# InternetMaximalism/stark-pure-rust

Measured on AMD Instinct MI355X. Metric: 2^24-pt NTT field-elems/sec, higher is better.
Workload: dtype u32x8 (BN254 Fr)

## Files before the change

### stark-pure-rust_amd/csrc/api.hip

```cpp
#include <new>
#include <string.h>

#include "internal.h"
#include "host_b2s.h"
#include "host_json.h"
#include "blake2s.h"

namespace stark {

stark_status hip_fail(stark_ctx* ctx, hipError_t e, const char* what) {
  if (ctx) {
    ctx->last_error = std::string(what) + ": " + hipGetErrorString(e);
  }
  return e == hipErrorOutOfMemory ? STARK_ERR_OOM : STARK_ERR_HIP;
}

bool poison_on() {
  static const bool on = [] {
    const char* v = getenv("STARK_POISON");
    return v && v[0] == '1';
  }();
  return on;
}
void poison_dev(void* p, size_t bytes) {
// ... 240 lines not shown

uint32_t stark_abi_version(void) { return STARK_ABI_VERSION; }
uint32_t stark_verify_simd_width(void) { return (uint32_t)b2s_paths_width(); }
uint32_t stark_json_simd_width(void) { return (uint32_t)json_simd_width(); }

stark_status stark_ctx_create(int device, stark_ctx** out) {
  if (!out) return STARK_ERR_BAD_ARG;
  *out = nullptr;
  int count = 0;
  if (hipGetDeviceCount(&count) != hipSuccess || device < 0 || device >= count) return STARK_ERR_NO_DEVICE;
  hipDeviceProp_t prop;
  if (hipGetDeviceProperties(&prop, device) != hipSuccess) return STARK_ERR_NO_DEVICE;
  if (strncmp(prop.gcnArchName, "gfx950", 6) != 0) return STARK_ERR_NO_DEVICE;
  stark_ctx* ctx = new (std::nothrow) stark_ctx();
  if (!ctx) return STARK_ERR_OOM;
  ctx->device = device;
  if (hipSetDevice(device) != hipSuccess || hipStreamCreateWithFlags(&ctx->stream, hipStreamNonBlocking) != hipSuccess) {
    delete ctx;
    return STARK_ERR_HIP;
  }
  *out = ctx;
  return STARK_OK;
}

void stark_ctx_destroy(stark_ctx* ctx) {
  if (!ctx) return;
  hipSetDevice(ctx->device);
  hipStreamSynchronize(ctx->stream);
  hipDeviceSynchronize();
  for (auto& kv : ctx->tw) {
    if (kv.second->d_lo) hipFree(kv.second->d_lo);
    if (kv.second->d_full) hipFree(kv.second->d_full);
    if (kv.second->d_full_s) hipFree(kv.second->d_full_s);
    for (hipEvent_t e : kv.second->full_ev)
      if (e) hipEventDestroy(e);
  }
  for (stark_merkle_tree*& t : ctx->trees) {
    stark_merkle_free(t);
    t = nullptr;
  }
  for (stark_merkle_tree* t : ctx->fri_trees) stark_merkle_free(t);
  for (void* p : ctx->pinned)
    if (p) hipHostFree(p);
  for (auto& kv : ctx->ext_idx)
    if (kv.second.ptr) hipFree(kv.second.ptr);
  for (auto& kv : ctx->post_tw) {
    if (kv.second.ptr) hipFree(kv.second.ptr);
    if (kv.second.ev) hipEventDestroy(kv.second.ev);
  }
  if (ctx->staged) hipEventDestroy(ctx->staged);
  if (ctx->ev_aux) hipEventDestroy(ctx->ev_aux);
  if (ctx->aux) hipStreamDestroy(ctx->aux);
  ctx->fri_trees.clear();
  for (DevBuf* b : {&ctx->scratch, &ctx->io, &ctx->io2, &ctx->inv_tmp, &ctx->fri_cols, &ctx->r1cs_arena, &ctx->trace_arena, &ctx->trace_raw, &ctx->fri_misc,
                     &ctx->lde_tmp, &ctx->verify_arena, &ctx->verify_lde, &ctx->ext_idx_tmp, &ctx->spot}) {
    if (b->ptr) hipFree(b->ptr);
    if (b->ev) hipEventDestroy(b->ev);
  }
  hipStreamDestroy(ctx->stream);
  delete ctx;
}

const char* stark_ctx_last_error(const stark_ctx* ctx) { return ctx ? ctx->last_error.c_str() : ""; }

stark_status stark_ctx_set_cache_limit(stark_ctx* ctx, size_t bytes) {
  if (!ctx) return STARK_ERR_BAD_ARG;
// ... 168 lines not shown
```

### stark-pure-rust_amd/csrc/internal.h

```cpp
#pragma once
#include <hip/hip_runtime.h>
#include <stdint.h>
#include <stdio.h>
#include <stdlib.h>

#include <chrono>

#include <functional>
#include <future>
#include <map>
#include <memory>
#include <string>
#include <tuple>
#include <vector>

#include "stark_hip.h"
#include "fp_dev.h"
#include "fp_host.h"
#include "host_pool.h"

namespace stark {

struct PhaseClock {
  bool on;
// ... 10 lines not shown
      return v && v[0] && v[0] != '0';
    }();
    return e;
  }
  void mark(const char* phase) {
    if (!on) return;
    const auto now = std::chrono::steady_clock::now();
    fprintf(stderr, "[stark]   %-28s %8.1f us (at %8.1f)\n", phase,
            std::chrono::duration<double, std::micro>(now - last).count(),
            std::chrono::duration<double, std::micro>(now - t0).count());
    last = now;
  }
};

struct DevBuf {
  void* ptr = nullptr;
  size_t bytes = 0;
  hipEvent_t ev = nullptr;
  hipStream_t last = nullptr;
};

struct Twiddles {
  uint32_t log_n = 0, kb = 0;
  fe* d_lo = nullptr;
  fe* d_hi = nullptr;
  fe* d_small = nullptr;
  fe* d_t16 = nullptr;
  fe* d_hi_s = nullptr;
  fe* d_t16_s = nullptr;
  uint32_t l16 = 0;
  uint32_t small_off[16] = {0};
  fe* d_full = nullptr;
  fe* d_full_s = nullptr;
  uint64_t full_used = 0, full_s_used = 0;
  hipEvent_t full_ev[2] = {nullptr, nullptr};
  hipStream_t full_fill[2] = {nullptr, nullptr};
  size_t base_bytes = 0;
  size_t n_small_pairs = 0;
  uint32_t* d_db = nullptr;
  uint32_t db_off[16] = {0};
  HostFp root;
  HostFp inv_n;
};

struct CacheBuf {
  void* ptr = nullptr;
  size_t bytes = 0;
  uint64_t used = 0;
  bool in_use = false;
  hipEvent_t ev = nullptr;
  hipStream_t fill = nullptr;
};

constexpr size_t kDefaultCacheLimit = (size_t)4 << 30;

}

struct stark_ctx {
  int device = 0;
  hipStream_t stream = nullptr;
  std::string last_error;
  stark::DevBuf scratch;
  stark::DevBuf io;
  stark::DevBuf io2;
  stark::DevBuf fri_cols;
  stark::DevBuf r1cs_arena;
  stark::DevBuf trace_arena;
  stark::DevBuf trace_raw;
  stark::DevBuf lde_tmp;
  stark::DevBuf verify_arena, verify_lde;
  stark::DevBuf ext_idx_tmp;
  stark::DevBuf inv_tmp;
  stark::DevBuf spot;
// ... 342 lines not shown
```

### stark-pure-rust_amd/csrc/ntt.hip

```cpp
#include <stdlib.h>

#include "fe_db.h"
#include "internal.h"

namespace stark {

struct ColTw {
  const fe* t16;
  const fe* lo;
  const fe* hi;
  const fe* full;
  uint32_t l16, kb;
  const fe* post;
};


__device__ __forceinline__ void shoup2(fe& r, fe& s, const fe& a, const fe& w, const fe& wq, const fe& c,
                                       const fe& x, const fe& xq) {
  r = fe_mul_shoup(a, w, wq);
  s = fe_mul_shoup(c, x, xq);
}
__device__ __forceinline__ void mul2(fe& r, fe& s, const fe& a, const fe& b, const fe& c, const fe& d) {
  fe_mul_lazy2(r, s, a, b, c, d);
}

__device__ __forceinline__ void bfly_lt2p(fe& x, fe& y, const fe& t) {
  fe_bfly_lazy_reduced(x, y, t);
}

__device__ __forceinline__ void sub2p(fe& t) {
  const P2Limbs q = p2_vgprs();
  asm("v_sub_co_u32 %0, vcc, %0, %8\n\t"
      "v_subb_co_u32 %1, vcc, %1, %9, vcc\n\t"
      "v_subb_co_u32 %2, vcc, %2, %10, vcc\n\t"
      "v_subb_co_u32 %3, vcc, %3, %11, vcc\n\t"
      "v_subb_co_u32 %4, vcc, %4, %12, vcc\n\t"
      "v_subb_co_u32 %5, vcc, %5, %13, vcc\n\t"
      "v_subb_co_u32 %6, vcc, %6, %14, vcc\n\t"
      "v_subb_co_u32 %7, vcc, %7, %15, vcc"
      : "+v"(t.w[0]), "+v"(t.w[1]), "+v"(t.w[2]), "+v"(t.w[3]), "+v"(t.w[4]), "+v"(t.w[5]), "+v"(t.w[6]),
        "+v"(t.w[7])
      : "v"(q.l[0]), "v"(q.l[1]), "v"(q.l[2]), "v"(q.l[3]), "v"(q.l[4]), "v"(q.l[5]), "v"(q.l[6]), "v"(q.l[7])
      : "vcc");
}
__device__ __forceinline__ void csub2p_top(fe& t) {
  if (t.w[7] > STARK_2P7) sub2p(t);
}
template <bool FAST>
__device__ __forceinline__ void bfly(fe& x, fe& y, const fe& t) {
  if (FAST) {
    csub2p_top(x);
    fe_bfly_lazy_reduced(x, y, t);
  } else {
    fe_bfly_lazy(x, y, t);
  }
}
template <bool FAST>
__device__ __forceinline__ void csub2p_t(fe& t) {
  if (FAST) csub2p_top(t);
  fe_csub2p(t);
}
template <bool FAST>
__device__ __forceinline__ void reduce_full(fe& t) {
  csub2p_t<FAST>(t);
  fe_reduce_once(t);
}

__device__ __forceinline__ const uint32_t* dbt(const uint32_t* sdb, uint32_t k) {
  return static_cast<const uint32_t*>(__builtin_assume_aligned(sdb + 72 * k + 4 * (k >> 3), 16));
}

enum : int { kColNone = 0, kColFull = 1, kColT16 = 2, kColTwoLevel = 3, kColSparse = 4 };

constexpr uint32_t kTileLog = 10;
constexpr uint32_t kPassThreads = (1u << kTileLog) / 4;

template <int LOG_R, int COL>
struct DbPlan {
  static constexpr bool on = LOG_R >= 4 && LOG_R <= 8;
  static constexpr bool four = LOG_R == 8 || (LOG_R == 7 && COL == kColSparse);
  static constexpr int s_end = on ? LOG_R - 2 : 0;
  static constexpr uint32_t stride = 4;
  static constexpr uint32_t entries = (on && !four) ? (1u << LOG_R) / (2 * stride) : 0;
  static constexpr uint32_t lds_fe = entries * 9 + entries / 16;
  static constexpr bool last = on && !four && LOG_R <= 7;
  static constexpr uint32_t full_entries = last ? (1u << LOG_R) / 2 : 0;
  static constexpr uint32_t full_fe = full_entries * 9 + full_entries / 16;
  static constexpr uint32_t shoup_fe = last ? 0 : four ? 2 * (1u << LOG_R) : (1u << LOG_R);
  static constexpr int occupancy = on ? 3 : 4;
};

typedef unsigned int u32x4_nt __attribute__((ext_vector_type(4)));
__device__ __forceinline__ fe fe_load_nt(const fe* p) {
  const u32x4_nt* q = reinterpret_cast<const u32x4_nt*>(p);
  const u32x4_nt lo = __builtin_nontemporal_load(q), hi = __builtin_nontemporal_load(q + 1);
  fe r;
  r.w[0] = lo.x; r.w[1] = lo.y; r.w[2] = lo.z; r.w[3] = lo.w;
  r.w[4] = hi.x; r.w[5] = hi.y; r.w[6] = hi.z; r.w[7] = hi.w;
  return r;
}
__device__ __forceinline__ void fe_store_nt(fe* p, const fe& v) {
  u32x4_nt* q = reinterpret_cast<u32x4_nt*>(p);
  __builtin_nontemporal_store(u32x4_nt{v.w[0], v.w[1], v.w[2], v.w[3]}, q);
  __builtin_nontemporal_store(u32x4_nt{v.w[4], v.w[5], v.w[6], v.w[7]}, q + 1);
}

struct XImage {
  fe* base;
  uint32_t n;
  __device__ __forceinline__ fe ld(uint32_t i) const {
    const uint4* v = reinterpret_cast<const uint4*>(base);
    const uint4 lo = v[i], hi = v[n + i];
    fe r;
    r.w[0] = lo.x; r.w[1] = lo.y; r.w[2] = lo.z; r.w[3] = lo.w;
    r.w[4] = hi.x; r.w[5] = hi.y; r.w[6] = hi.z; r.w[7] = hi.w;
    return r;
  }
  __device__ __forceinline__ void st(uint32_t i, const fe& x) const {
    uint4* v = reinterpret_cast<uint4*>(base);
    v[i] = make_uint4(x.w[0], x.w[1], x.w[2], x.w[3]);
    v[n + i] = make_uint4(x.w[4], x.w[5], x.w[6], x.w[7]);
  }
};

template <int LOG_R, int COL>
__global__ __launch_bounds__(kPassThreads, (DbPlan<LOG_R, COL>::occupancy)) void ntt_pass_kernel(
    const fe* __restrict__ in, fe* __restrict__ out, uint32_t log_n, uint32_t log_ns, uint32_t log_b, ColTw ct,
    const fe* __restrict__ small, const uint32_t* __restrict__ db, fe scale, int do_scale, uint32_t log_tiles,
    uint32_t total_tiles, Sparse sp) {
  constexpr uint32_t R = 1u << LOG_R;
  using DB = DbPlan<LOG_R, COL>;
  constexpr bool FAST = LOG_R == 6;
  extern __shared__ __attribute__((aligned(16))) fe lds[];
  fe* sm = lds;
  uint32_t* sdb = reinterpret_cast<uint32_t*>(lds + DB::shoup_fe);
  fe* X = lds + DB::shoup_fe + DB::lds_fe;
  const uint32_t B = 1u << log_b;
  const XImage XI{X, B << LOG_R};
  const uint32_t nthr = (B << LOG_R) >> 2;
  const uint32_t tid = threadIdx.x;
  const bool active = tid < nthr;
  const uint32_t log_cols = log_n - LOG_R;
  const size_t ns_mask = ((size_t)1 << log_ns) - 1;
  const uint32_t tile_mask = (1u << log_tiles) - 1;
  const uint32_t tile = blockIdx.x;
  if (tile >= total_tiles) return;

  uint32_t eb[4], er[4];
#pragma unroll
  for (int t = 0; t < 4; ++t) {
    const uint32_t e = tid + (uint32_t)t * nthr;
    eb[t] = e & (B - 1);
    er[t] = e >> log_b;
  }
  const uint32_t b = tid & (B - 1);
  const uint32_t q = tid >> log_b;

  const uint32_t live_rows = R >> sp.skip, nz_rows = R >> sp.zero_log;
  const uint32_t log_in = sp.zero_log ? sp.log_in : log_n;
  fe v[4];
  if (active) {
    const fe* src = in + ((size_t)(tile >> log_tiles) << log_in) + ((size_t)(tile & tile_mask) << log_b);
#pragma unroll
    for (int t = 0; t < 4; ++t)
      v[t] = er[t] < nz_rows ? fe_load(src + eb[t] + ((size_t)er[t] << log_cols)) : fe_zero();
  }

  {
    constexpr uint32_t kSm = 2 * DB::shoup_fe, kDb = DB::on ? DB::entries * 18 : 0;
    const uint4* db4 = reinterpret_cast<const uint4*>(db);
    const uint4* small4 = reinterpret_cast<const uint4*>(small);
    uint4* sm4 = reinterpret_cast<uint4*>(sm);
    uint4* sdb4 = reinterpret_cast<uint4*>(sdb);
    auto db_src = [&](uint32_t k) { const uint32_t e = k / 18; return (e * DB::stride) * 18 + (k - e * 18); };
    auto db_dst = [&](uint32_t k) { return k + ((k / 18) >> 3); };
    if (blockDim.x == kPassThreads) {
      constexpr uint32_t nSm = (kSm + kPassThreads - 1) / kPassThreads, nDb = (kDb + kPassThreads - 1) / kPassThreads;
      auto in_sm = [&](uint32_t i) { return (i + 1) * kPassThreads <= kSm || tid + i * kPassThreads < kSm; };
      auto in_db = [&](uint32_t i) { return (i + 1) * kPassThreads <= kDb || tid + i * kPassThreads < kDb; };
      uint4 ts[nSm ? nSm : 1], td[nDb ? nDb : 1];
#pragma unroll
      for (uint32_t i = 0; i < nSm; ++i)
        if (in_sm(i)) ts[i] = small4[tid + i * kPassThreads];
#pragma unroll
      for (uint32_t i = 0; i < nDb; ++i)
        if (in_db(i)) td[i] = db4[db_src(tid + i * kPassThreads)];
#pragma unroll
      for (uint32_t i = 0; i < nSm; ++i)
        if (in_sm(i)) sm4[tid + i * kPassThreads] = ts[i];
#pragma unroll
      for (uint32_t i = 0; i < nDb; ++i)
        if (in_db(i)) sdb4[db_dst(tid + i * kPassThreads)] = td[i];
    } else {
      for (uint32_t k = tid; k < kSm; k += blockDim.x) sm4[k] = small4[k];
      for (uint32_t k = tid; k < kDb; k += blockDim.x) sdb4[db_dst(k)] = db4[db_src(k)];
    }
  }
  const size_t boff = (size_t)(tile >> log_tiles) << log_n;
  const size_t j0 = (size_t)(tile & tile_mask) << log_b;

  if (active) {
    if (COL != kColNone && COL != kColSparse) {
      const uint32_t lnr = log_ns + LOG_R;
      fe tw[4];
      if (COL == kColFull) {
#pragma unroll
        for (int t = 0; t < 4; ++t) tw[t] = fe_load_nt(ct.full + ((((j0 + eb[t]) & ns_mask) << LOG_R) + er[t]));
        mul2(v[0], v[1], v[0], tw[0], v[1], tw[1]);
        mul2(v[2], v[3], v[2], tw[2], v[3], tw[3]);
      } else if (COL == kColT16) {
        const fe* e[4];
#pragma unroll
        for (int t = 0; t < 4; ++t) {
          const uint64_t k = ((uint64_t)((j0 + eb[t]) & ns_mask) * er[t]) & (((uint64_t)1 << lnr) - 1);
          e[t] = ct.t16 + 2 * (k << (ct.l16 - lnr));
        }
        shoup2(v[0], v[1], v[0], e[0][0], e[0][1], v[1], e[1][0], e[1][1]);
        shoup2(v[2], v[3], v[2], e[2][0], e[2][1], v[3], e[3][0], e[3][1]);
      } else {
        const uint32_t unit = log_n - lnr;
#pragma unroll
        for (int t = 0; t < 4; ++t) {
          const uint64_t ex = ((uint64_t)((j0 + eb[t]) & ns_mask) * er[t]) << unit;
          tw[t] = fe_mul(ct.lo[ex & (((uint64_t)1 << ct.kb) - 1)], ct.hi[ex >> ct.kb]);
        }
        mul2(v[0], v[1], v[0], tw[0], v[1], tw[1]);
        mul2(v[2], v[3], v[2], tw[2], v[3], tw[3]);
// ... 1 lines not shown
    }
    if (sp.skip == 0) {
      if ((LOG_R & 1) == 0) {
        bfly_lt2p(v[0], v[2], v[2]);
        bfly_lt2p(v[1], v[3], v[3]);
        fe t3;
        if (DB::on) {
          t3 = fe_mul_db(v[3], db + 72u * (1u << (LOG_R - 2)));
        } else {
          const uint32_t ic = 2 * (1u << (LOG_R - 2));
          t3 = fe_mul_shoup(v[3], small[ic], small[ic + 1]);
        }
        fe_csub2p(v[1]);
        bfly<FAST>(v[0], v[1], v[1]);
        bfly<FAST>(v[2], v[3], t3);
      } else {
        bfly_lt2p(v[0], v[2], v[2]);
        bfly_lt2p(v[1], v[3], v[3]);
      }
#pragma unroll
      for (int t = 0; t < 4; ++t) {
        const uint32_t rr = __builtin_bitreverse32(er[t]) >> (32 - LOG_R);
        XI.st((rr << log_b) + eb[t], v[t]);
      }
    } else {
#pragma unroll
      for (int t = 0; t < 4; ++t) {
        if (er[t] >= live_rows) continue;
        const uint32_t rr = __builtin_bitreverse32(er[t]) >> (32 - LOG_R);
        for (uint32_t k = 0; k < (1u << sp.skip); ++k) XI.st(((rr + k) << log_b) + eb[t], v[t]);
      }
    }
  }
  __syncthreads();

  int s = sp.skip ? (int)sp.skip : (LOG_R & 1) ? 1 : 2;
  constexpr int kS0 = (LOG_R & 1) ? 1 : 2;
  if (LOG_R >= 5 && s == kS0) {
    if (active) {
      const uint32_t lq = LOG_R + log_b - 2 - kS0;
      const uint32_t jj = tid >> lq;
      const uint32_t rest = tid & ((1u << lq) - 1);
      const uint32_t i0 = ((((rest >> log_b) << (kS0 + 2)) + jj) << log_b) + (rest & (B - 1));
      const uint32_t st = (1u << kS0) << log_b;
      fe x0 = XI.ld(i0), x1 = XI.ld(i0 + st), x2 = XI.ld(i0 + 2 * st), x3 = XI.ld(i0 + 3 * st);
      if (jj == 0) {
        csub2p_t<FAST>(x1);
        csub2p_t<FAST>(x3);
        bfly<FAST>(x0, x1, x1);
        bfly<FAST>(x2, x3, x3);
        fe t3;
        if (DB::on) {
          t3 = fe_mul_db(x3, db + 72u * (1u << (LOG_R - 2)));
        } else {
          const uint32_t ic = 2 * (1u << (LOG_R - 2));
          t3 = fe_mul_shoup(x3, sm[ic], sm[ic + 1]);
        }
        csub2p_t<FAST>(x2);
        bfly<FAST>(x0, x2, x2);
        bfly<FAST>(x1, x3, t3);
      } else if (DB::on && DB::s_end > kS0 && lq >= 6) {
        const uint32_t ju = __builtin_amdgcn_readfirstlane(jj);
        const uint32_t* wa = db + 72u * (ju << (LOG_R - 1 - kS0));
        const fe t1 = fe_mul_db(x1, wa);
        fe t3 = fe_mul_db(x3, wa);
        bfly<FAST>(x0, x1, t1);
// ... 5 lines not shown
      } else if (DB::on && DB::s_end > kS0) {
        constexpr uint32_t S = DB::stride;
        auto tab = [&](uint32_t e) { return DB::four ? db + 72u * e : dbt(sdb, e / S); };
        const uint32_t* wa = tab(jj << (LOG_R - 1 - kS0));
        const fe t1 = fe_mul_db(x1, wa);
        fe t3 = fe_mul_db(x3, wa);
        bfly<FAST>(x0, x1, t1);
        bfly<FAST>(x2, x3, t3);
        const fe t2 = fe_mul_db(x2, tab(jj << (LOG_R - 2 - kS0)));
        t3 = fe_mul_db(x3, tab((jj + (1u << kS0)) << (LOG_R - 2 - kS0)));
        bfly<FAST>(x0, x2, t2);
        bfly<FAST>(x1, x3, t3);
      } else {
        fe t1, t3;
        const uint32_t ia = 2 * (jj << (LOG_R - 1 - kS0));
        const fe ta = sm[ia], taq = sm[ia + 1];
        shoup2(t1, t3, x1, ta, taq, x3, ta, taq);
        bfly<FAST>(x0, x1, t1);
        bfly<FAST>(x2, x3, t3);
        const uint32_t ic = 2 * ((jj + (1u << kS0)) << (LOG_R - 2 - kS0));
        const fe tc = sm[ic], tcq = sm[ic + 1];
        const uint32_t ib = 2 * (jj << (LOG_R - 2 - kS0));
        const fe t2 = fe_mul_shoup(x2, sm[ib], sm[ib + 1]);
        t3 = fe_mul_shoup(x3, tc, tcq);
        bfly<FAST>(x0, x2, t2);
        bfly<FAST>(x1, x3, t3);
      }
      XI.st(i0, x0);
      XI.st(i0 + 2 * st, x2);
      XI.st(i0 + st, x1);
      XI.st(i0 + 3 * st, x3);
    }
    __syncthreads();
    s = kS0 + 2;
  }
  bool kept = false;
  fe yl[4];
  constexpr uint32_t LT = LOG_R >= 4 ? LOG_R - 4 : 0;
  if (DB::four && s == (int)LT) {
    if (active) {
      const uint32_t t = q & ((1u << LT) - 1), a = q >> LT;
      const uint32_t i0 = (((a << (LT + 2)) + t) << log_b) + b, st = (1u << LT) << log_b;
      fe x[4];
      const bool unit0 = ((64u >> log_b) <= (1u << LT) ? __builtin_amdgcn_readfirstlane(a) : a) == 0;
#pragma unroll
      for (int k = 0; k < 4; ++k) {
        const fe v = XI.ld(i0 + k * st);
        if (k == 0 && unit0) {
          x[0] = v;
          fe_csub2p(x[0]);
          continue;
        }
        const uint32_t e = (__builtin_bitreverse32((a << 2) + k) >> 28) * t;
        x[k] = fe_mul_shoup(v, sm[2 * e], sm[2 * e + 1]);
      }
      bfly_lt2p(x[0], x[1], x[1]);
      bfly_lt2p(x[2], x[3], x[3]);
      const fe t3 = fe_mul_db(x[3], db + 72u * (1u << (LOG_R - 2)));
      fe_csub2p(x[2]);
      bfly<FAST>(x[0], x[2], x[2]);
      bfly<FAST>(x[1], x[3], t3);
#pragma unroll
      for (int k = 0; k < 4; ++k) XI.st(i0 + k * st, x[k]);
    }
    __syncthreads();
    if (active) {
      const uint32_t i0 = (q << log_b) + b, st = (R / 4) << log_b;
      fe x0 = XI.ld(i0), x1 = XI.ld(i0 + st), x2 = XI.ld(i0 + 2 * st), x3 = XI.ld(i0 + 3 * st);
      auto step = [&](const uint32_t a) {
        if (a == 0) {
          csub2p_t<FAST>(x1);
          csub2p_t<FAST>(x3);
          bfly<FAST>(x0, x1, x1);
          bfly<FAST>(x2, x3, x3);
          const fe t3 = fe_mul_db(x3, db + 72u * (1u << (LOG_R - 2)));
          csub2p_t<FAST>(x2);
          bfly<FAST>(x0, x2, x2);
          bfly<FAST>(x1, x3, t3);
        } else {
          const uint32_t* wa = db + 72u * (a << (LOG_R - 3));
          const fe t1 = fe_mul_db(x1, wa);
          fe t3 = fe_mul_db(x3, wa);
          bfly<FAST>(x0, x1, t1);
          bfly<FAST>(x2, x3, t3);
          const fe t2 = fe_mul_db(x2, db + 72u * (a << LT));
          t3 = fe_mul_db(x3, db + 72u * ((a + 4) << LT));
          bfly<FAST>(x0, x2, t2);
          bfly<FAST>(x1, x3, t3);
        }
      };
      if ((64u >> log_b) <= (1u << LT))
        step(__builtin_amdgcn_readfirstlane(q >> LT));
      else
        step(q >> LT);
      yl[0] = x0;
      yl[1] = x1;
      yl[2] = x2;
      yl[3] = x3;
    }
    kept = true;
    s = LOG_R;
  }
  if (DB::on && !DB::four) {
#pragma unroll 1
    for (; s < DB::s_end; s += 2) {
      if (active) {
        const uint32_t m = 1u << s;
        const uint32_t jj = q & (m - 1);
        const uint32_t base = ((q >> s) << (s + 2)) + jj;
        fe x0 = XI.ld((base << log_b) + b);
        fe x1 = XI.ld(((base + m) << log_b) + b);
        fe x2 = XI.ld(((base + 2 * m) << log_b) + b);
        fe x3 = XI.ld(((base + 3 * m) << log_b) + b);
        constexpr uint32_t S = DB::stride;
        const uint32_t* wa = dbt(sdb, (jj << (LOG_R - 1 - s)) / S);
        const fe t1 = fe_mul_db(x1, wa);
        fe t3 = fe_mul_db(x3, wa);
        bfly<FAST>(x0, x1, t1);
        bfly<FAST>(x2, x3, t3);
        const fe t2 = fe_mul_db(x2, dbt(sdb, (jj << (LOG_R - 2 - s)) / S));
        t3 = fe_mul_db(x3, dbt(sdb, ((jj + m) << (LOG_R - 2 - s)) / S));
        bfly<FAST>(x0, x2, t2);
        bfly<FAST>(x1, x3, t3);
        XI.st((base << log_b) + b, x0);
        XI.st(((base + 2 * m) << log_b) + b, x2);
        XI.st(((base + m) << log_b) + b, x1);
        XI.st(((base + 3 * m) << log_b) + b, x3);
      }
      __syncthreads();
    }
  }
// ... 209 lines not shown
template <int COL>
size_t db_lds_fe_c(uint32_t log_r) {
  switch (log_r) {
    case 4: return DbPlan<4, COL>::lds_fe + DbPlan<4, COL>::shoup_fe;
    case 5: return DbPlan<5, COL>::lds_fe + DbPlan<5, COL>::shoup_fe;
    case 6: return DbPlan<6, COL>::lds_fe + DbPlan<6, COL>::shoup_fe;
    case 7: return DbPlan<7, COL>::lds_fe + DbPlan<7, COL>::shoup_fe;
    case 8: return DbPlan<8, COL>::lds_fe + DbPlan<8, COL>::shoup_fe;
    case 9: return DbPlan<9, COL>::lds_fe + DbPlan<9, COL>::shoup_fe;
    default: return (size_t)1 << log_r;
  }
}
size_t db_lds_fe(uint32_t log_r, int col) {
  switch (col) {
    case kColNone: return db_lds_fe_c<kColNone>(log_r);
    case kColSparse: return db_lds_fe_c<kColSparse>(log_r);
    case kColFull: return db_lds_fe_c<kColFull>(log_r);
    case kColT16: return db_lds_fe_c<kColT16>(log_r);
    default: return db_lds_fe_c<kColTwoLevel>(log_r);
  }
}

template <int LOG_R>
pass_fn pass_kernel_r(int col) {
  switch (col) {
    case kColNone: return ntt_pass_kernel<LOG_R, kColNone>;
    case kColSparse: return ntt_pass_kernel<LOG_R, kColSparse>;
    case kColFull: return ntt_pass_kernel<LOG_R, kColFull>;
    case kColT16: return ntt_pass_kernel<LOG_R, kColT16>;
    default: return ntt_pass_kernel<LOG_R, kColTwoLevel>;
  }
}

pass_fn pass_kernel(uint32_t log_r, int col) {
  switch (log_r) {
    case 2: return pass_kernel_r<2>(col);
    case 3: return pass_kernel_r<3>(col);
    case 4: return pass_kernel_r<4>(col);
    case 5: return pass_kernel_r<5>(col);
    case 6: return pass_kernel_r<6>(col);
    case 7: return pass_kernel_r<7>(col);
    case 8: return pass_kernel_r<8>(col);
    case 9: return pass_kernel_r<9>(col);
    default: return nullptr;
  }
}

}

stark_status get_twiddles(stark_ctx* ctx, const uint64_t root[4], uint32_t log_n, const Twiddles** out) {
  const FieldHost& F = FieldHost::get();
  if (log_n > 28) return STARK_ERR_BAD_LENGTH;
  auto key = std::make_tuple(root[0], root[1], root[2], root[3], log_n);
  auto it = ctx->tw.find(key);
  if (it != ctx->tw.end()) {
    *out = it->second.get();
    return STARK_OK;
  }
  const HostFp w = F.from_canonical(root);
  HostFp t = w;
  if (log_n == 0) {
    if (!FieldHost::eq(w, F.one())) return STARK_ERR_BAD_ROOT;
  } else {
    for (uint32_t i = 1; i < log_n; ++i) t = F.mul(t, t);
    const HostFp minus_one = F.sub(F.zero(), F.one());
    if (!FieldHost::eq(t, minus_one)) return STARK_ERR_BAD_ROOT;
  }
  auto tw = std::make_unique<Twiddles>();
  tw->log_n = log_n;
  tw->kb = (log_n + 1) / 2;
  tw->root = w;
  tw->inv_n = F.inv(F.from_u64((uint64_t)1 << log_n));
  const size_t n_lo = (size_t)1 << tw->kb, n_hi = (size_t)1 << (log_n - tw->kb);
  std::vector<fe> h_lo(n_lo), h_hi(n_hi);
  HostFp acc = F.one();
  for (size_t i = 0; i < n_lo; ++i) {
    h_lo[i] = to_dev(acc);
    acc = F.mul(acc, w);
  }
  const HostFp step = acc;
  acc = F.one();
// ... 49 lines not shown
  tw->n_small_pairs = h_small.size() / 2;
  std::vector<uint32_t> h_db;
  for (uint32_t l = 1; l <= kMaxLogR && l <= log_n; ++l) {
    tw->db_off[l] = (uint32_t)h_db.size();
    const HostFp wr = F.pow_u64(w, (uint64_t)1 << (log_n - l));
    HostFp a = F.one();
    for (uint32_t k = 0; k < (1u << (l - 1)); ++k) {
      uint32_t t[72];
      db_table(a, t);
      h_db.insert(h_db.end(), t, t + 72);
      a = F.mul(a, wr);
    }
  }
  if (h_db.empty()) h_db.resize(72, 0);
  const size_t db_fe = h_db.size() / 8;
  const size_t bytes = (n_lo + 2 * n_hi + h_small.size() + 4 * n16 + db_fe) * sizeof(fe);
  void* d = nullptr;
  if (hipMalloc(&d, bytes) != hipSuccess) return STARK_ERR_OOM;
  tw->d_lo = (fe*)d;
  tw->d_hi = tw->d_lo + n_lo;
  tw->d_small = tw->d_hi + n_hi;
  tw->d_t16 = tw->d_small + h_small.size();
  tw->d_hi_s = tw->d_t16 + 2 * n16;
  tw->d_t16_s = tw->d_hi_s + n_hi;
  tw->d_db = reinterpret_cast<uint32_t*>(tw->d_t16_s + 2 * n16);
  tw->base_bytes = bytes;
  STARK_HIP(ctx, hipMemcpy(tw->d_lo, h_lo.data(), n_lo * sizeof(fe), hipMemcpyHostToDevice));
  STARK_HIP(ctx, hipMemcpy(tw->d_hi, h_hi.data(), n_hi * sizeof(fe), hipMemcpyHostToDevice));
  STARK_HIP(ctx, hipMemcpy(tw->d_small, h_small.data(), h_small.size() * sizeof(fe), hipMemcpyHostToDevice));
  STARK_HIP(ctx, hipMemcpy(tw->d_t16, h_t16.data(), 2 * n16 * sizeof(fe), hipMemcpyHostToDevice));
  STARK_HIP(ctx, hipMemcpy(tw->d_hi_s, h_hi_s.data(), n_hi * sizeof(fe), hipMemcpyHostToDevice));
  STARK_HIP(ctx, hipMemcpy(tw->d_t16_s, h_t16_s.data(), 2 * n16 * sizeof(fe), hipMemcpyHostToDevice));
  STARK_HIP(ctx, hipMemcpy(tw->d_db, h_db.data(), h_db.size() * sizeof(uint32_t), hipMemcpyHostToDevice));
  *out = tw.get();
  ctx->tw.emplace(key, std::move(tw));
  return STARK_OK;
}

__global__ void full_tw_kernel(const fe* __restrict__ lo, const fe* __restrict__ hi, uint32_t kb, uint32_t log_r,
                               uint64_t n, fe scale, int do_scale, fe* __restrict__ out) {
  const uint64_t g = (uint64_t)blockIdx.x * blockDim.x + threadIdx.x;
  if (g >= n) return;
  const uint64_t e = (g >> log_r) * (g & (((uint64_t)1 << log_r) - 1));
  fe t = fe_mul(lo[e & (((uint64_t)1 << kb) - 1)], hi[e >> kb]);
  if (do_scale) t = fe_mul(t, scale);
  fe_store(out + g, t);
}

static stark_status full_table(stark_ctx* ctx, const Twiddles& tw_c, uint32_t log_r, bool scaled, hipStream_t stream,
                               const fe** out) {
  Twiddles& tw = const_cast<Twiddles&>(tw_c);
  fe*& slot = scaled ? tw.d_full_s : tw.d_full;
  const int d = scaled ? 1 : 0;
  (scaled ? tw.full_s_used : tw.full_used) = ++ctx->cache_clock;
  if (!slot) {
    const uint64_t n = (uint64_t)1 << tw.log_n;
    void* p = nullptr;
    if (!cache_reserve(ctx, n * sizeof(fe), false) || hipMalloc(&p, n * sizeof(fe)) != hipSuccess) {
      hipGetLastError();
      *out = nullptr;
      return STARK_OK;
    }
    hipLaunchKernelGGL(full_tw_kernel, dim3((unsigned)((n + 255) / 256)), dim3(256), 0, stream, tw.d_lo, tw.d_hi,
                       tw.kb, log_r, n, to_dev(tw.inv_n), scaled ? 1 : 0, (fe*)p);
    STARK_HIP(ctx, hipGetLastError());
    STARK_TRY(fill_mark(ctx, tw.full_ev[d], tw.full_fill[d], stream));
    slot = (fe*)p;
  } else {
    STARK_TRY(fill_wait(ctx, tw.full_ev[d], tw.full_fill[d], stream));
  }
  *out = slot;
  return STARK_OK;
}

}

extern "C" uint32_t stark_ntt_plan(uint32_t log_n, uint32_t* log_r, uint32_t cap) {
  if (log_n < 2 || log_n > 28) return 0;
  const stark::PassPlan p = stark::plan_passes(log_n);
  for (int i = 0; i < p.n_pass && (uint32_t)i < cap; ++i) log_r[i] = p.log_r[i];
  return (uint32_t)p.n_pass;
}

namespace stark {

uint32_t ntt_first_log_r(uint32_t log_n) { return log_n < 2 ? log_n : plan_passes(log_n).log_r[0]; }

stark_status ntt_device(stark_ctx* ctx, fe* d_data, uint32_t log_n, uint32_t batch, const Twiddles& tw,
                        bool inverse, hipStream_t stream, const fe* post) {
  return ntt_device_from(ctx, nullptr, 0, d_data, log_n, batch, tw, inverse, stream, post);
}

stark_status ntt_device_from(stark_ctx* ctx, const fe* src, uint32_t zero_log, fe* d_data, uint32_t log_n,
                             uint32_t batch, const Twiddles& tw, bool inverse, hipStream_t stream, const fe* post) {
  if (batch == 0) return STARK_OK;
  if (src && zero_log > log_n) return STARK_ERR_BAD_ARG;
  if (src && (zero_log == 0 || log_n < 2 || zero_log > plan_passes(log_n).log_r[0])) {
    const uint64_t total = (uint64_t)batch << log_n;
    hipLaunchKernelGGL(pad_kernel, dim3((unsigned)((total + 255) / 256)), dim3(256), 0, stream, src, d_data,
                       log_n - zero_log, log_n, total);
    STARK_HIP(ctx, hipGetLastError());
    src = nullptr;
  }
  if (((uint64_t)batch << log_n) > ((uint64_t)1 << 34)) return STARK_ERR_BAD_ARG;
  const size_t n = (size_t)1 << log_n;
  const fe scale = to_dev(tw.inv_n);
  if (log_n == 0) return STARK_OK;
  if (log_n == 1) {
    if (post) return STARK_ERR_BAD_ARG;
    hipLaunchKernelGGL(ntt2_kernel, dim3(batch), dim3(1), 0, stream, d_data, scale, inverse ? 1 : 0);
    STARK_HIP(ctx, hipGetLastError());
    return STARK_OK;
  }
  const PassPlan plan = plan_passes(log_n);
  fe* scratch = nullptr;
  stark_status st = STARK_OK;
  if (plan.n_pass > 1) {
    st = ensure_buf(ctx, ctx->scratch, n * batch * sizeof(fe));
    if (st != STARK_OK) return st;
    STARK_TRY(buf_acquire(ctx, ctx->scratch, stream));
    scratch = (fe*)ctx->scratch.ptr;
  }
  const fe* cur = src ? src : d_data;
  uint32_t log_ns = 0;
  for (int p = 0; p < plan.n_pass; ++p) {
    const uint32_t lr = plan.log_r[p];
    const bool last = p == plan.n_pass - 1;
    fe* dst = last ? d_data : (cur == d_data ? scratch : d_data);
    Sparse sp{0, 0, log_n};
    if (p == 0 && src) {
      uint32_t k = zero_log < lr ? zero_log : lr;
      if ((k & 1) != (lr & 1)) --k;
      sp = Sparse{k, zero_log, log_n - zero_log};
    }
    const uint32_t lb = choose_log_b_impl(log_n, lr, kTileLog);
    const uint32_t elems = 1u << (lr + lb);
    const uint32_t threads = elems / 4 < 64 ? 64 : elems / 4;
    const uint32_t log_tiles = log_n - lr - lb;
    const uint64_t total = (uint64_t)batch << log_tiles;
    const bool fold = inverse && last && log_ns > 0;
    const fe* full = nullptr;
    if (last && log_ns > 0 && log_n > tw.l16 && log_n >= 17 && log_n <= 26) {
      st = full_table(ctx, tw, lr, fold, stream, &full);
      if (st != STARK_OK) return st;
    }
    ColTw ct{fold ? tw.d_t16_s : tw.d_t16, tw.d_lo, fold ? tw.d_hi_s : tw.d_hi, full, tw.l16, tw.kb,
             last ? post : nullptr};
    const int col = log_ns == 0 ? (sp.skip ? kColSparse : kColNone)
                    : full ? kColFull : log_ns + lr <= tw.l16 ? kColT16 : kColTwoLevel;
    const size_t image = std::max((size_t)elems, db_full_fe(lr, col));
    const size_t lds = (image + db_lds_fe(lr, col)) * sizeof(fe);
    hipLaunchKernelGGL(pass_kernel(lr, col), dim3((unsigned)total), dim3(threads), lds, stream, cur, dst, log_n,
                       log_ns, lb, ct, tw.d_small + tw.small_off[lr], tw.d_db + tw.db_off[lr], scale,
                       (inverse && last && !fold) ? 1 : 0, log_tiles, (uint32_t)total, sp);
    STARK_HIP(ctx, hipGetLastError());
    cur = dst;
    log_ns += lr;
  }
  if (scratch) buf_release(ctx, ctx->scratch, stream);
  return STARK_OK;
}

stark_status ntt_first_pass_tmajor(stark_ctx* ctx, const fe* src, uint32_t zero_log, fe* out, uint32_t log_n,
                                   uint32_t batch, const Twiddles& tw, hipStream_t stream, uint32_t* log_t) {
  if (!src || log_n < 2 || zero_log == 0 || batch == 0 || tw.log_n != log_n) return STARK_ERR_BAD_ARG;
  if (((uint64_t)batch << log_n) > ((uint64_t)1 << 34)) return STARK_ERR_BAD_ARG;
  const uint32_t lr = plan_passes(log_n).log_r[0];
  if (zero_log > lr) return STARK_ERR_BAD_ARG;
  uint32_t k = zero_log;
  if ((k & 1) != (lr & 1)) --k;
  const Sparse sp{k, zero_log, log_n - zero_log};
  const uint32_t lb = choose_log_b_impl(log_n, lr, kTileLog);
  const uint32_t elems = 1u << (lr + lb);
  const uint32_t threads = elems / 4 < 64 ? 64 : elems / 4;
  const uint32_t log_tiles = log_n - lr - lb;
  const uint64_t total = (uint64_t)batch << log_tiles;
  const int col = sp.skip ? kColSparse : kColNone;
  const ColTw ct{tw.d_t16, tw.d_lo, tw.d_hi, nullptr, tw.l16, tw.kb, nullptr};
  const size_t image = std::max((size_t)elems, db_full_fe(lr, col));
  const size_t lds = (image + db_lds_fe(lr, col)) * sizeof(fe);
  hipLaunchKernelGGL(pass_kernel(lr, col), dim3((unsigned)total), dim3(threads), lds, stream, src, out, log_n,
                     log_n - lr, lb, ct, tw.d_small + tw.small_off[lr], tw.d_db + tw.db_off[lr], to_dev(tw.inv_n), 0,
                     log_tiles, (uint32_t)total, sp);
  STARK_HIP(ctx, hipGetLastError());
  *log_t = lr;
  return STARK_OK;
}
// ... 3 lines not shown
```

Baseline: 11.37 billion.

## Fuse inter-pass twiddle multiply into radix-256 producer passes for 2^24 NTT

Moves the column twiddle multiplication of the following pass into the preceding dense radix-2^8 pass. A staged variant builds per-tile twiddles in LDS from the t16 table, plus a residual table multiply. A streamed variant reads a precomputed fused full-size table. This lets the consumer pass run without column twiddles, and by default only the staged mode is enabled, for log_n == 24. It adds residual-table setup, extra multiplies in the producer pass and more code complexity.

```diff
diff --git a/stark-pure-rust_amd/csrc/api.hip b/stark-pure-rust_amd/csrc/api.hip
--- a/stark-pure-rust_amd/csrc/api.hip
+++ b/stark-pure-rust_amd/csrc/api.hip
@@ -296,6 +296,8 @@
     if (kv.second->d_lo) hipFree(kv.second->d_lo);
     if (kv.second->d_full) hipFree(kv.second->d_full);
     if (kv.second->d_full_s) hipFree(kv.second->d_full_s);
+    for (uint32_t* r : kv.second->d_res)
+      if (r) hipFree(r);
     for (hipEvent_t e : kv.second->full_ev)
       if (e) hipEventDestroy(e);
   }
diff --git a/stark-pure-rust_amd/csrc/internal.h b/stark-pure-rust_amd/csrc/internal.h
--- a/stark-pure-rust_amd/csrc/internal.h
+++ b/stark-pure-rust_amd/csrc/internal.h
@@ -66,6 +66,8 @@
   uint32_t small_off[16] = {0};
   fe* d_full = nullptr;
   fe* d_full_s = nullptr;
+  static constexpr uint32_t kFullFused = 0x100;
+  uint32_t full_kind[2] = {0, 0};
   uint64_t full_used = 0, full_s_used = 0;
   hipEvent_t full_ev[2] = {nullptr, nullptr};
   hipStream_t full_fill[2] = {nullptr, nullptr};
@@ -73,6 +75,7 @@
   size_t n_small_pairs = 0;
   uint32_t* d_db = nullptr;
   uint32_t db_off[16] = {0};
+  uint32_t* d_res[13] = {nullptr};
   HostFp root;
   HostFp inv_n;
 };
diff --git a/stark-pure-rust_amd/csrc/ntt.hip b/stark-pure-rust_amd/csrc/ntt.hip
--- a/stark-pure-rust_amd/csrc/ntt.hip
+++ b/stark-pure-rust_amd/csrc/ntt.hip
@@ -12,6 +12,10 @@
   const fe* full;
   uint32_t l16, kb;
   const fe* post;
+  const uint32_t* res;
+  const fe* fused;
+  uint32_t log_rp;
+  uint32_t log_q;
 };
 
 
@@ -72,6 +76,8 @@
 
 enum : int { kColNone = 0, kColFull = 1, kColT16 = 2, kColTwoLevel = 3, kColSparse = 4 };
 
+enum : int { kFuseNone = 0, kFuseStaged = 1, kFuseStreamed = 2 };
+
 constexpr uint32_t kTileLog = 10;
 constexpr uint32_t kPassThreads = (1u << kTileLog) / 4;
 
@@ -123,7 +129,7 @@
   }
 };
 
-template <int LOG_R, int COL>
+template <int LOG_R, int COL, int FUSE = kFuseNone>
 __global__ __launch_bounds__(kPassThreads, (DbPlan<LOG_R, COL>::occupancy)) void ntt_pass_kernel(
     const fe* __restrict__ in, fe* __restrict__ out, uint32_t log_n, uint32_t log_ns, uint32_t log_b, ColTw ct,
     const fe* __restrict__ small, const uint32_t* __restrict__ db, fe scale, int do_scale, uint32_t log_tiles,
@@ -131,6 +137,8 @@
   constexpr uint32_t R = 1u << LOG_R;
   using DB = DbPlan<LOG_R, COL>;
   constexpr bool FAST = LOG_R == 6;
+  static_assert(FUSE == kFuseNone || (LOG_R == 8 && (COL == kColNone || (COL == kColT16 && FUSE == kFuseStreamed))),
+                "fused producers are the dense radix-2^8 passes");
   extern __shared__ __attribute__((aligned(16))) fe lds[];
   fe* sm = lds;
   uint32_t* sdb = reinterpret_cast<uint32_t*>(lds + DB::shoup_fe);
@@ -145,6 +153,7 @@
   const uint32_t tile_mask = (1u << log_tiles) - 1;
   const uint32_t tile = blockIdx.x;
   if (tile >= total_tiles) return;
+  const uint32_t rp = FUSE ? ((tile & tile_mask) << log_b) >> ct.log_q : 0;
 
   uint32_t eb[4], er[4];
 #pragma unroll
@@ -167,13 +176,23 @@
   }
 
   {
-    constexpr uint32_t kSm = 2 * DB::shoup_fe, kDb = DB::on ? DB::entries * 18 : 0;
+    constexpr uint32_t kSm = FUSE == kFuseStreamed ? 0 : 2 * DB::shoup_fe, kDb = DB::on ? DB::entries * 18 : 0;
     const uint4* db4 = reinterpret_cast<const uint4*>(db);
     const uint4* small4 = reinterpret_cast<const uint4*>(small);
     uint4* sm4 = reinterpret_cast<uint4*>(sm);
     uint4* sdb4 = reinterpret_cast<uint4*>(sdb);
     auto db_src = [&](uint32_t k) { const uint32_t e = k / 18; return (e * DB::stride) * 18 + (k - e * 18); };
     auto db_dst = [&](uint32_t k) { return k + ((k / 18) >> 3); };
+    auto sm_src = [&](uint32_t u) -> const uint4* {
+      if (FUSE == kFuseStaged) {
+        const uint32_t slot = u >> 2, t = slot & (R / 16 - 1);
+        const uint32_t r1 = __builtin_bitreverse32(slot / (R / 16)) >> 28;
+        const uint32_t lnp = LOG_R + ct.log_rp;
+        const uint32_t idx = (((r1 * t) << ct.log_rp) + t * rp) & ((1u << lnp) - 1);
+        return reinterpret_cast<const uint4*>(ct.t16) + ((((size_t)idx << (ct.l16 - lnp)) << 2) + (u & 3));
+      }
+      return small4 + u;
+    };
     if (blockDim.x == kPassThreads) {
       constexpr uint32_t nSm = (kSm + kPassThreads - 1) / kPassThreads, nDb = (kDb + kPassThreads - 1) / kPassThreads;
       auto in_sm = [&](uint32_t i) { return (i + 1) * kPassThreads <= kSm || tid + i * kPassThreads < kSm; };
@@ -181,7 +200,7 @@
       uint4 ts[nSm ? nSm : 1], td[nDb ? nDb : 1];
 #pragma unroll
       for (uint32_t i = 0; i < nSm; ++i)
-        if (in_sm(i)) ts[i] = small4[tid + i * kPassThreads];
+        if (in_sm(i)) ts[i] = *sm_src(tid + i * kPassThreads);
 #pragma unroll
       for (uint32_t i = 0; i < nDb; ++i)
         if (in_db(i)) td[i] = db4[db_src(tid + i * kPassThreads)];
@@ -192,7 +211,7 @@
       for (uint32_t i = 0; i < nDb; ++i)
         if (in_db(i)) sdb4[db_dst(tid + i * kPassThreads)] = td[i];
     } else {
-      for (uint32_t k = tid; k < kSm; k += blockDim.x) sm4[k] = small4[k];
+      for (uint32_t k = tid; k < kSm; k += blockDim.x) sm4[k] = *sm_src(k);
       for (uint32_t k = tid; k < kDb; k += blockDim.x) sdb4[db_dst(k)] = db4[db_src(k)];
     }
   }
@@ -260,6 +279,15 @@
       }
     }
   }
+  fe ftw[4];
+  auto load_ftw = [&]() {
+    const fe* f = ct.fused + ((size_t)(tile & tile_mask) << (LOG_R + log_b)) + tid;
+#pragma unroll
+    for (int k = 0; k < 4; ++k) ftw[k] = fe_load_nt(f + (uint32_t)k * nthr);
+  };
+#ifdef STARK_FUSED_TW_EARLY
+  if (FUSE == kFuseStreamed && active) load_ftw();
+#endif
   __syncthreads();
 
   int s = sp.skip ? (int)sp.skip : (LOG_R & 1) ? 1 : 2;
@@ -331,6 +359,9 @@
       XI.st(i0 + 3 * st, x3);
     }
     __syncthreads();
+#ifndef STARK_FUSED_TW_EARLY
+    if (FUSE == kFuseStreamed && active) load_ftw();
+#endif
     s = kS0 + 2;
   }
   bool kept = false;
@@ -341,10 +372,21 @@
       const uint32_t t = q & ((1u << LT) - 1), a = q >> LT;
       const uint32_t i0 = (((a << (LT + 2)) + t) << log_b) + b, st = (1u << LT) << log_b;
       fe x[4];
-      const bool unit0 = ((64u >> log_b) <= (1u << LT) ? __builtin_amdgcn_readfirstlane(a) : a) == 0;
+      const bool unit0 = FUSE == kFuseNone && ((64u >> log_b) <= (1u << LT) ? __builtin_amdgcn_readfirstlane(a) : a) == 0;
+      if (FUSE == kFuseStreamed) {
+        const fe v0 = XI.ld(i0), v1 = XI.ld(i0 + st), v2 = XI.ld(i0 + 2 * st), v3 = XI.ld(i0 + 3 * st);
+        mul2(x[0], x[1], v0, ftw[0], v1, ftw[1]);
+        mul2(x[2], x[3], v2, ftw[2], v3, ftw[3]);
+      }
 #pragma unroll
       for (int k = 0; k < 4; ++k) {
+        if (FUSE == kFuseStreamed) break;
         const fe v = XI.ld(i0 + k * st);
+        if (FUSE == kFuseStaged) {
+          const uint32_t slot = (((a << 2) + k) << LT) + t;
+          x[k] = fe_mul_shoup(v, sm[2 * slot], sm[2 * slot + 1]);
+          continue;
+        }
         if (k == 0 && unit0) {
           x[0] = v;
           fe_csub2p(x[0]);
@@ -396,6 +438,17 @@
       yl[1] = x1;
       yl[2] = x2;
       yl[3] = x3;
+      if (FUSE != kFuseNone) {
+        const uint32_t k2 = __builtin_amdgcn_readfirstlane(q >> LT);
+#pragma unroll
+        for (uint32_t kk = 0; kk < 4; ++kk) {
+          const uint32_t e = (k2 + 4 * kk) * rp;
+          if (e == 0)
+            fe_csub2p(yl[kk]);
+          else
+            yl[kk] = fe_mul_db(yl[kk], ct.res + 72u * e);
+        }
+      }
     }
     kept = true;
     s = LOG_R;
@@ -671,7 +724,14 @@
   }
 }
 
-pass_fn pass_kernel(uint32_t log_r, int col) {
+pass_fn pass_kernel(uint32_t log_r, int col, int fuse = kFuseNone) {
+  if (fuse != kFuseNone) {
+    if (log_r != 8) return nullptr;
+    if (fuse == kFuseStaged) return col == kColNone ? ntt_pass_kernel<8, kColNone, kFuseStaged> : nullptr;
+    return col == kColNone  ? ntt_pass_kernel<8, kColNone, kFuseStreamed>
+           : col == kColT16 ? ntt_pass_kernel<8, kColT16, kFuseStreamed>
+                            : nullptr;
+  }
   switch (log_r) {
     case 2: return pass_kernel_r<2>(col);
     case 3: return pass_kernel_r<3>(col);
@@ -685,7 +745,47 @@
   }
 }
 
-}
+enum : int { kFuseAuto = 0, kFuseAll = 1, kFuseForceStreamed = 2, kFuseOff = 3 };
+
+inline uint32_t fuse_default(uint32_t log_n) {
+#ifdef STARK_FUSE_ALL_SIZES
+  return (1u << kFuseStaged) | (1u << kFuseStreamed);
+#endif
+#ifdef STARK_FUSE_ONLY
+  return log_n == 24 ? 1u << STARK_FUSE_ONLY : 0;
+#endif
+  return log_n == 24 ? 1u << kFuseStaged : 0;
+}
+
+void fuse_modes(const PassPlan& plan, uint32_t log_n, uint32_t l16, int policy, bool dense_first, int fz[8]) {
+  for (int p = 0; p < 8; ++p) fz[p] = kFuseNone;
+  const uint32_t allowed = policy == kFuseAuto ? fuse_default(log_n) : ~0u;
+  if (policy == kFuseOff || !allowed) return;
+  uint32_t log_ns = 0;
+  for (int p = 0; p + 1 < plan.n_pass; log_ns += plan.log_r[p], ++p) {
+    const uint32_t lr = plan.log_r[p], lrn = plan.log_r[p + 1];
+    if (lr != 8 || lrn > 8 || log_n < lr + lrn) continue;
+    const uint32_t lb = choose_log_b_impl(log_n, lr, kTileLog);
+    if (lb != kTileLog - 8 || log_n - lr - lrn < lb) continue;
+    if (p == 0 && !dense_first) continue;
+    const bool fused_in = p > 0 && fz[p - 1] != kFuseNone;
+    const bool staged = p == 0 && lr + lrn <= l16;
+    const bool streamed = p + 2 == plan.n_pass && lrn == 8 && log_n >= 18 && log_n <= 26 &&
+                          (p == 0 || fused_in || log_ns + lr <= l16);
+    if (policy == kFuseForceStreamed)
+      fz[p] = streamed ? kFuseStreamed : staged ? kFuseStaged : kFuseNone;
+    else
+      fz[p] = staged ? kFuseStaged : streamed ? kFuseStreamed : kFuseNone;
+    if (!(allowed >> fz[p] & 1)) fz[p] = kFuseNone;
+  }
+}
+
+}
+
+static stark_status res_table(stark_ctx* ctx, Twiddles& tw, uint32_t m);
+static stark_status ntt_device_plan(stark_ctx* ctx, const fe* src, uint32_t zero_log, fe* d_data, uint32_t log_n,
+                                    uint32_t batch, const Twiddles& tw, bool inverse, hipStream_t stream,
+                                    const fe* post, const PassPlan& plan, int policy, uint32_t* used = nullptr);
 
 stark_status get_twiddles(stark_ctx* ctx, const uint64_t root[4], uint32_t log_n, const Twiddles** out) {
   const FieldHost& F = FieldHost::get();
@@ -801,6 +901,21 @@
   STARK_HIP(ctx, hipMemcpy(tw->d_hi_s, h_hi_s.data(), n_hi * sizeof(fe), hipMemcpyHostToDevice));
   STARK_HIP(ctx, hipMemcpy(tw->d_t16_s, h_t16_s.data(), 2 * n16 * sizeof(fe), hipMemcpyHostToDevice));
   STARK_HIP(ctx, hipMemcpy(tw->d_db, h_db.data(), h_db.size() * sizeof(uint32_t), hipMemcpyHostToDevice));
+  if (log_n >= 2) {
+    const PassPlan plan = plan_passes(log_n);
+    int fz[8];
+    fuse_modes(plan, log_n, tw->l16, kFuseAuto, true, fz);
+    for (int p = 0; p + 1 < plan.n_pass; ++p)
+      if (fz[p] != kFuseNone) {
+        const stark_status st = res_table(ctx, *tw, 4 + plan.log_r[p + 1]);
+        if (st != STARK_OK) {
+          for (uint32_t* r : tw->d_res)
+            if (r) hipFree(r);
+          hipFree(tw->d_lo);
+          return st;
+        }
+      }
+  }
   *out = tw.get();
   ctx->tw.emplace(key, std::move(tw));
   return STARK_OK;
@@ -816,12 +931,35 @@
   fe_store(out + g, t);
 }
 
-static stark_status full_table(stark_ctx* ctx, const Twiddles& tw_c, uint32_t log_r, bool scaled, hipStream_t stream,
+__global__ void fused_tw_kernel(const fe* __restrict__ lo, const fe* __restrict__ hi, uint32_t kb, uint32_t log_n,
+                                fe scale, int do_scale, fe* __restrict__ out) {
+  const uint64_t g = (uint64_t)blockIdx.x * blockDim.x + threadIdx.x;
+  if (g >> log_n) return;
+  const uint32_t log_ns = log_n - 16;
+  const uint32_t tid = (uint32_t)g & 255, kk = ((uint32_t)g >> 8) & 3;
+  const uint64_t j = ((g >> 10) << 2) + (tid & 3);
+  const uint32_t q = tid >> 2, k1 = q & 15;
+  const uint32_t r1 = __builtin_bitreverse32(((q >> 4) << 2) + kk) >> 28;
+  const uint64_t c = j & (((uint64_t)1 << log_ns) - 1), rp = j >> log_ns;
+  const uint64_t e = (((uint64_t)(r1 * k1) << (log_n - 8)) + (c + ((uint64_t)k1 << log_ns)) * rp) &
+                     (((uint64_t)1 << log_n) - 1);
+  fe t = fe_mul(lo[e & (((uint64_t)1 << kb) - 1)], hi[e >> kb]);
+  if (do_scale) t = fe_mul(t, scale);
+  fe_store(out + g, t);
+}
+
+static stark_status full_table(stark_ctx* ctx, const Twiddles& tw_c, uint32_t kind, bool scaled, hipStream_t stream,
                                const fe** out) {
   Twiddles& tw = const_cast<Twiddles&>(tw_c);
   fe*& slot = scaled ? tw.d_full_s : tw.d_full;
   const int d = scaled ? 1 : 0;
   (scaled ? tw.full_s_used : tw.full_used) = ++ctx->cache_clock;
+  if (slot && tw.full_kind[d] != kind) {
+    STARK_HIP(ctx, hipDeviceSynchronize());
+    hipFree(slot);
+    slot = nullptr;
+    tw.full_fill[d] = nullptr;
+  }
   if (!slot) {
     const uint64_t n = (uint64_t)1 << tw.log_n;
     void* p = nullptr;
@@ -830,15 +968,44 @@
       *out = nullptr;
       return STARK_OK;
     }
-    hipLaunchKernelGGL(full_tw_kernel, dim3((unsigned)((n + 255) / 256)), dim3(256), 0, stream, tw.d_lo, tw.d_hi,
-                       tw.kb, log_r, n, to_dev(tw.inv_n), scaled ? 1 : 0, (fe*)p);
+    if (kind == Twiddles::kFullFused)
+      hipLaunchKernelGGL(fused_tw_kernel, dim3((unsigned)((n + 255) / 256)), dim3(256), 0, stream, tw.d_lo, tw.d_hi,
+                         tw.kb, tw.log_n, to_dev(tw.inv_n), scaled ? 1 : 0, (fe*)p);
+    else
+      hipLaunchKernelGGL(full_tw_kernel, dim3((unsigned)((n + 255) / 256)), dim3(256), 0, stream, tw.d_lo, tw.d_hi,
+                         tw.kb, kind, n, to_dev(tw.inv_n), scaled ? 1 : 0, (fe*)p);
     STARK_HIP(ctx, hipGetLastError());
     STARK_TRY(fill_mark(ctx, tw.full_ev[d], tw.full_fill[d], stream));
     slot = (fe*)p;
+    tw.full_kind[d] = kind;
   } else {
     STARK_TRY(fill_wait(ctx, tw.full_ev[d], tw.full_fill[d], stream));
   }
   *out = slot;
+  return STARK_OK;
+}
+
+static stark_status res_table(stark_ctx* ctx, Twiddles& tw, uint32_t m) {
+  if (m > 12 || m > tw.log_n) return STARK_ERR_BAD_ARG;
+  if (tw.d_res[m]) return STARK_OK;
+  const FieldHost& F = FieldHost::get();
+  const size_t cnt = (size_t)1 << m;
+  std::vector<uint32_t> h(72 * cnt);
+  const HostFp wm = F.pow_u64(tw.root, (uint64_t)1 << (tw.log_n - m));
+  HostFp a = F.one();
+  for (size_t e = 0; e < cnt; ++e) {
+    db_table(a, &h[72 * e]);
+    a = F.mul(a, wm);
+  }
+  void* d = nullptr;
+  if (hipMalloc(&d, h.size() * sizeof(uint32_t)) != hipSuccess) return STARK_ERR_OOM;
+  const hipError_t e = hipMemcpy(d, h.data(), h.size() * sizeof(uint32_t), hipMemcpyHostToDevice);
+  if (e != hipSuccess) {
+    hipFree(d);
+    return hip_fail(ctx, e, "hipMemcpy(residual table)");
+  }
+  tw.d_res[m] = (uint32_t*)d;
+  tw.base_bytes += h.size() * sizeof(uint32_t);
   return STARK_OK;
 }
 
@@ -851,6 +1018,34 @@
   return (uint32_t)p.n_pass;
 }
 
+extern "C" int stark_test_ntt_plan(stark_ctx* ctx, uint64_t* d_data, uint32_t log_n, uint32_t batch,
+                                   const uint64_t root[4], int inverse, const uint32_t* log_r, uint32_t n_pass,
+                                   int policy, void* stream, uint32_t* used) {
+  using namespace stark;
+  if (!ctx || !d_data || !root || !log_r || n_pass == 0 || n_pass > 8 || log_n < 2 || log_n > 28 || policy < 0 ||
+      policy > 3)
+    return STARK_ERR_BAD_ARG;
+  PassPlan plan;
+  plan.n_pass = (int)n_pass;
+  uint32_t sum = 0;
+  for (uint32_t i = 0; i < n_pass; ++i) {
+    if (log_r[i] < 2 || log_r[i] > kMaxLogR) return STARK_ERR_BAD_ARG;
+    plan.log_r[i] = log_r[i];
+    sum += log_r[i];
+  }
+  if (sum != log_n) return STARK_ERR_BAD_ARG;
+  STARK_HIP(ctx, hipSetDevice(ctx->device));
+  const FieldHost& F = FieldHost::get();
+  uint64_t use_root[4];
+  memcpy(use_root, root, 32);
+  if (inverse) F.to_canonical(F.inv(F.from_canonical(root)), use_root);
+  if (used) *used = 0;
+  const Twiddles* tw = nullptr;
+  STARK_TRY(get_twiddles(ctx, use_root, log_n, &tw));
+  return ntt_device_plan(ctx, nullptr, 0, (fe*)d_data, log_n, batch, *tw, inverse != 0, pick_stream(ctx, stream),
+                         nullptr, plan, policy, used);
+}
+
 namespace stark {
 
 uint32_t ntt_first_log_r(uint32_t log_n) { return log_n < 2 ? log_n : plan_passes(log_n).log_r[0]; }
@@ -862,9 +1057,16 @@
 
 stark_status ntt_device_from(stark_ctx* ctx, const fe* src, uint32_t zero_log, fe* d_data, uint32_t log_n,
                              uint32_t batch, const Twiddles& tw, bool inverse, hipStream_t stream, const fe* post) {
+  return ntt_device_plan(ctx, src, zero_log, d_data, log_n, batch, tw, inverse, stream, post,
+                         log_n >= 2 ? plan_passes(log_n) : PassPlan(), kFuseAuto);
+}
+
+static stark_status ntt_device_plan(stark_ctx* ctx, const fe* src, uint32_t zero_log, fe* d_data, uint32_t log_n,
+                                    uint32_t batch, const Twiddles& tw, bool inverse, hipStream_t stream,
+                                    const fe* post, const PassPlan& plan, int policy, uint32_t* used) {
   if (batch == 0) return STARK_OK;
   if (src && zero_log > log_n) return STARK_ERR_BAD_ARG;
-  if (src && (zero_log == 0 || log_n < 2 || zero_log > plan_passes(log_n).log_r[0])) {
+  if (src && (zero_log == 0 || log_n < 2 || zero_log > plan.log_r[0])) {
     const uint64_t total = (uint64_t)batch << log_n;
     hipLaunchKernelGGL(pad_kernel, dim3((unsigned)((total + 255) / 256)), dim3(256), 0, stream, src, d_data,
                        log_n - zero_log, log_n, total);
@@ -881,7 +1083,19 @@
     STARK_HIP(ctx, hipGetLastError());
     return STARK_OK;
   }
-  const PassPlan plan = plan_passes(log_n);
+  int fz[8];
+  fuse_modes(plan, log_n, tw.l16, policy, src == nullptr, fz);
+  const fe* fused_tab = nullptr;
+  for (int p = 0; p + 1 < plan.n_pass; ++p)
+    if (fz[p] == kFuseStreamed) {
+      STARK_TRY(full_table(ctx, tw, Twiddles::kFullFused, inverse, stream, &fused_tab));
+      if (!fused_tab)
+        for (int& f : fz) f = kFuseNone;
+    }
+  if (used)
+    for (int p = 0; p + 1 < plan.n_pass; ++p) *used |= (uint32_t)fz[p] << (2 * p);
+  for (int p = 0; p + 1 < plan.n_pass; ++p)
+    if (fz[p] != kFuseNone) STARK_TRY(res_table(ctx, const_cast<Twiddles&>(tw), 4 + plan.log_r[p + 1]));
   fe* scratch = nullptr;
   stark_status st = STARK_OK;
   if (plan.n_pass > 1) {
@@ -907,21 +1121,31 @@
     const uint32_t threads = elems / 4 < 64 ? 64 : elems / 4;
     const uint32_t log_tiles = log_n - lr - lb;
     const uint64_t total = (uint64_t)batch << log_tiles;
-    const bool fold = inverse && last && log_ns > 0;
+    const bool fused_in = p > 0 && fz[p - 1] != kFuseNone;
+    const int fuse = last ? kFuseNone : fz[p];
+    const bool fold = inverse && last && log_ns > 0 && !fused_in;
     const fe* full = nullptr;
-    if (last && log_ns > 0 && log_n > tw.l16 && log_n >= 17 && log_n <= 26) {
+    if (last && log_ns > 0 && !fused_in && log_n > tw.l16 && log_n >= 17 && log_n <= 26) {
       st = full_table(ctx, tw, lr, fold, stream, &full);
       if (st != STARK_OK) return st;
     }
     ColTw ct{fold ? tw.d_t16_s : tw.d_t16, tw.d_lo, fold ? tw.d_hi_s : tw.d_hi, full, tw.l16, tw.kb,
-             last ? post : nullptr};
-    const int col = log_ns == 0 ? (sp.skip ? kColSparse : kColNone)
+             last ? post : nullptr, nullptr, nullptr, 0, 0};
+    if (fuse != kFuseNone) {
+      ct.res = tw.d_res[4 + plan.log_r[p + 1]];
+      ct.fused = fuse == kFuseStreamed ? fused_tab : nullptr;
+      ct.log_rp = plan.log_r[p + 1];
+      ct.log_q = log_n - lr - plan.log_r[p + 1];
+    }
+    const int col = (log_ns == 0 || fused_in) ? (sp.skip ? kColSparse : kColNone)
                     : full ? kColFull : log_ns + lr <= tw.l16 ? kColT16 : kColTwoLevel;
     const size_t image = std::max((size_t)elems, db_full_fe(lr, col));
     const size_t lds = (image + db_lds_fe(lr, col)) * sizeof(fe);
-    hipLaunchKernelGGL(pass_kernel(lr, col), dim3((unsigned)total), dim3(threads), lds, stream, cur, dst, log_n,
+    const pass_fn fn = pass_kernel(lr, col, fuse);
+    if (!fn) return STARK_ERR_BAD_ARG;
+    hipLaunchKernelGGL(fn, dim3((unsigned)total), dim3(threads), lds, stream, cur, dst, log_n,
                        log_ns, lb, ct, tw.d_small + tw.small_off[lr], tw.d_db + tw.db_off[lr], scale,
-                       (inverse && last && !fold) ? 1 : 0, log_tiles, (uint32_t)total, sp);
+                       (inverse && last && !fold && !fused_in) ? 1 : 0, log_tiles, (uint32_t)total, sp);
     STARK_HIP(ctx, hipGetLastError());
     cur = dst;
     log_ns += lr;
```

After: 11.68 billion, median of 6. +2.8%, better.
